# certfhe/CSGN

Hardware: AMD Instinct MI355X
Metric: ciphertext-mults/sec (N=1247, 1024-term operands) (higher is better)
Workload: dtype u64

## Files before the change

csgn_amd/batch.py:

```python
from __future__ import annotations

import ctypes as C
from typing import Optional, Tuple

import numpy as np
import torch

from . import capi
from .capi import check


def _ptr(t: Optional[torch.Tensor]) -> int:
    return 0 if t is None else t.data_ptr()


class HipPath:

    def __init__(self, device: int = 0):
        self.lib = capi.load_library()
        if not torch.cuda.is_available():
            raise capi.CsgnError(capi.CSGN_ERR_NO_DEVICE,
                                 "torch sees no GPU; csgn_amd has no CPU fallback")
        torch.cuda.set_device(device)
        check(self.lib.csgn_init(device))
# ... 775 lines not shown
            out = torch.empty(max(batch, 1), dtype=torch.int64, device=self.device)
        check(self.lib.csgn_uint_decrypt(n_bits, batch, w, h_planes, h_terms, h_off, h_total, h_max, _ptr(mask),
                                         _ptr(out), self.stream))
        return out[:batch]

    def decrypt_combined_uniform(self, n_bits: int, batch: int, t1: int, t2: int, left: torch.Tensor,
                                 right: torch.Tensor, mask: torch.Tensor, product: bool) -> torch.Tensor:
        bits = torch.empty(max(batch, 1), dtype=torch.uint8, device=self.device)
        scratch = torch.empty(int(self.lib.csgn_decrypt_combined_scratch_bytes(batch, t1, t2)),
                              dtype=torch.uint8, device=self.device)
        fn = self.lib.csgn_decrypt_product_uniform if product else self.lib.csgn_decrypt_sum_uniform
        check(fn(n_bits, batch, t1, t2, _ptr(left), _ptr(right), _ptr(mask), _ptr(bits), _ptr(scratch),
                 self.stream))
        return bits[:batch]

    def compact_ragged(self, n_bits: int, words: torch.Tensor, off: torch.Tensor,
                       total_terms: Optional[int] = None, max_terms: int = 0,
                       out: Optional[torch.Tensor] = None, off_out: Optional[torch.Tensor] = None,
                       scratch: Optional[torch.Tensor] = None,
                       sync: bool = True) -> Tuple[torch.Tensor, torch.Tensor]:
        batch = off.numel() - 1
        dl = self.default_len(n_bits)
        if total_terms is None:
            total_terms = int(self.download(off[-1:])[0])
        if out is None:
            out = self.empty_words(max(total_terms * dl, 1))
        if off_out is None:
            off_out = self.empty_words(batch + 1)
        if scratch is None:
            scratch = torch.empty(int(self.lib.csgn_compact_scratch_bytes(n_bits, batch, total_terms)),
# ... 98 lines not shown
```

csgn_amd/capi.py:

```python
from __future__ import annotations

import ctypes as C
import os
from typing import Optional

PKG = os.path.dirname(os.path.abspath(__file__))
_LIB_PATH = os.path.join(PKG, "lib", "libcsgn_hip.so")

CSGN_OK = 0
CSGN_ERR_INVALID = -1
CSGN_ERR_UNSUPPORTED = -2
CSGN_ERR_NO_DEVICE = -3
CSGN_ERR_HIP = -4

CSGN_GATE_NOT, CSGN_GATE_XNOR, CSGN_GATE_NAND, CSGN_GATE_OR, CSGN_GATE_NOR, CSGN_GATE_MUX, \
    CSGN_GATE_ADD_PLAIN, CSGN_GATE_MUL_PLAIN = range(1, 9)

CSGN_UINT_ADD_HALF, CSGN_UINT_ADD_FULL, CSGN_UINT_EQ_STEP, CSGN_UINT_LT_FIRST, CSGN_UINT_LT_STEP = range(1, 6)
CSGN_UINT_PLAIN_EQ, CSGN_UINT_PLAIN_NE, CSGN_UINT_PLAIN_LT, CSGN_UINT_PLAIN_LE, CSGN_UINT_PLAIN_GT, \
    CSGN_UINT_PLAIN_GE = range(1, 7)

u64 = C.c_uint64
vp = C.c_void_p

# ... 35 lines not shown
    "csgn_mul_plan_trust": (C.c_int, [vp, C.c_int]),
    "csgn_mul_ragged_async_plan_words": (u64, [u64]),
    "csgn_mul_ragged_async": (C.c_int, [u64, u64, vp, vp, vp, vp, vp, vp, u64, vp, vp]),
    "csgn_mul_ragged_async_result": (C.c_int, [vp, C.POINTER(u64 * 5), vp]),
    "csgn_add_uniform": (C.c_int, [u64, u64, u64, u64, vp, vp, vp, vp]),
    "csgn_add_ragged": (C.c_int, [u64, u64, vp, vp, vp, vp, vp, vp, u64, vp]),
    "csgn_small_ops": (C.c_int, [u64, u64, vp, vp]),
    "csgn_add_ragged_bounded": (C.c_int, [u64, u64, u64, u64, vp, vp, vp, vp, vp, vp, u64, vp]),
    "csgn_decrypt_scratch_bytes": (C.c_size_t, [u64, u64]),
    "csgn_decrypt_uniform": (C.c_int, [u64, u64, u64, vp, vp, vp, vp, vp]),
    "csgn_decrypt_ragged": (C.c_int, [u64, u64, u64, vp, vp, vp, vp, vp, vp]),
    "csgn_decrypt_ragged_bounded": (C.c_int, [u64, u64, u64, u64, vp, vp, vp, vp, vp, vp]),
    "csgn_decrypt_combined_scratch_bytes": (C.c_size_t, [u64, u64, u64]),
    "csgn_decrypt_product_uniform": (C.c_int, [u64, u64, u64, u64, vp, vp, vp, vp, vp, vp]),
    "csgn_decrypt_sum_uniform": (C.c_int, [u64, u64, u64, u64, vp, vp, vp, vp, vp, vp]),
    "csgn_compact_scratch_bytes": (C.c_size_t, [u64, u64, u64]),
    "csgn_compact_ragged": (C.c_int, [u64, u64, u64, u64, vp, vp, vp, vp, vp, vp]),
    "csgn_encrypt_explicit": (C.c_int, [u64, u64, u64, vp, vp, vp, vp, vp, vp, vp]),
    "csgn_rng_from_os": (C.c_int, [vp, C.c_uint32]),
    "csgn_rng_from_seed": (C.c_int, [vp, u64, C.c_uint32]),
    "csgn_encrypt_keyed_layout": (C.c_int, [u64, C.POINTER(C.c_uint32), C.POINTER(C.c_uint32), C.POINTER(C.c_uint32)]),
    "csgn_encrypt_keyed": (C.c_int, [u64, u64, u64, u64, vp, vp, vp, vp, vp, vp]),
    "csgn_encrypt_mul_keyed": (C.c_int, [u64, u64, u64, u64, vp, vp, vp, vp, vp, vp, vp, vp, vp]),
    "csgn_encrypt_device_rng": (C.c_int, [u64, u64, u64, vp, vp, vp, u64, vp, vp]),
    "csgn_permute_uniform": (C.c_int, [u64, u64, u64, C.c_int, vp, vp, vp, vp]),
    "csgn_bitlen_scratch_bytes": (C.c_size_t, [u64]),
    "csgn_decrypt_bitlen": (C.c_int, [u64, u64, u64, vp, vp, vp, vp, vp, vp]),
    "csgn_permute_bitlen": (C.c_int, [u64, u64, vp, vp, vp, vp, vp, vp]),
    "csgn_synth_fill": (C.c_int, [u64, u64, u64, u64, vp, vp]),
    "csgn_digest": (C.c_int, [vp, u64, u64, vp, vp]),
# ... 2 lines not shown
    "csgn_circuit_input": (C.c_int, [vp, u64, C.POINTER(C.c_uint32)]),
    "csgn_circuit_input_ragged": (C.c_int, [vp, vp, C.POINTER(C.c_uint32)]),
    "csgn_circuit_add": (C.c_int, [vp, C.c_uint32, C.c_uint32, C.POINTER(C.c_uint32)]),
    "csgn_circuit_mul": (C.c_int, [vp, C.c_uint32, C.c_uint32, C.POINTER(C.c_uint32)]),
    "csgn_circuit_decrypt": (C.c_int, [vp, C.c_uint32, vp, C.POINTER(C.c_uint32)]),
    "csgn_circuit_compact": (C.c_int, [vp, C.c_uint32, C.POINTER(C.c_uint32)]),
    "csgn_circuit_permute": (C.c_int, [vp, C.c_uint32, vp, C.POINTER(C.c_uint32)]),
    "csgn_circuit_encrypt": (C.c_int, [vp, u64, vp, vp, vp, vp, u64, C.POINTER(C.c_uint32)]),
    "csgn_circuit_encrypt_mul": (C.c_int, [vp, u64, vp, vp, vp, vp, vp, vp, u64, C.POINTER(C.c_uint32), C.POINTER(C.c_uint32)]),
    "csgn_circuit_epoch": (u64, [vp]),
    "csgn_circuit_node_key": (C.c_int, [vp, vp]),
    "csgn_circuit_optimize": (C.c_int, [vp, C.c_uint32]),
    "csgn_circuit_output": (C.c_int, [vp, C.c_uint32]),
    "csgn_circuit_block_bytes": (u64, [vp]),
    "csgn_circuit_stats": (C.c_int, [vp, vp]),
    "csgn_circuit_plan_json": (C.c_int, [vp, vp, C.c_size_t]),
    "csgn_circuit_build": (C.c_int, [vp]),
    "csgn_circuit_value": (vp, [vp, C.c_uint32]),
    "csgn_circuit_value_terms": (u64, [vp, C.c_uint32]),
    "csgn_circuit_value_total_terms": (u64, [vp, C.c_uint32]),
    "csgn_circuit_value_offsets": (vp, [vp, C.c_uint32]),
    "csgn_circuit_bits": (vp, [vp, C.c_uint32]),
    "csgn_circuit_run": (C.c_int, [vp, vp]),
    "csgn_mul_uniform_kernel": (C.c_char_p, [u64, u64, u64, u64]),
    "csgn_gate_terms": (u64, [C.c_int, u64, u64, u64]),
    "csgn_gate_uniform_kernel": (C.c_char_p, [u64, C.c_int, u64, u64, u64, u64]),
    "csgn_gate_uniform": (C.c_int, [u64, C.c_int, u64, u64, u64, u64, vp, vp, vp, vp, vp, vp]),
    "csgn_const_fill": (C.c_int, [u64, u64, vp, C.c_int, vp, vp]),
    "csgn_uint_step_terms": (u64, [C.c_int, C.c_int, u64, u64, u64]),
    "csgn_uint_step_kernel": (C.c_char_p, [u64, C.c_int, u64, u64, u64, u64]),
# ... 269 lines not shown
```

csgn_amd/csrc/csgn_capi.hip:

```cpp
#include "csgn_capi_util.h"
#include "csgn_device.h"
#include "csgn_tuning.h"

#include <sys/random.h>

#include <cerrno>
#include <cstdarg>
#include <vector>
#include <cstdio>
#include <cstring>

namespace csgn {
namespace capi {

thread_local char g_err[512] = "";

int fail(int code, const char *fmt, ...)
{
    va_list ap;
    va_start(ap, fmt);
    vsnprintf(g_err, sizeof(g_err), fmt, ap);
    va_end(ap);
    return code;
}
// ... 728 lines not shown
    return CSGN_OK;
}

int csgn_decrypt_product_uniform(uint64_t n_bits, uint64_t batch, uint64_t t1, uint64_t t2,
                                 const uint64_t *d_left, const uint64_t *d_right,
                                 const uint64_t *d_mask, uint8_t *d_bits, void *d_scratch, void *stream)
{
    return decrypt_combined_uniform(true, n_bits, batch, t1, t2, d_left, d_right, d_mask, d_bits, d_scratch, stream);
}

int csgn_decrypt_sum_uniform(uint64_t n_bits, uint64_t batch, uint64_t t1, uint64_t t2,
                             const uint64_t *d_left, const uint64_t *d_right,
                             const uint64_t *d_mask, uint8_t *d_bits, void *d_scratch, void *stream)
{
    return decrypt_combined_uniform(false, n_bits, batch, t1, t2, d_left, d_right, d_mask, d_bits, d_scratch, stream);
}

size_t csgn_compact_scratch_bytes(uint64_t n_bits, uint64_t batch, uint64_t total_terms)
{
    if (n_bits == 0 || !csgn::compact_supported(n_bits))
        return 0;
    return csgn::compact_scratch_bytes(n_bits, batch, total_terms);
}

int csgn_compact_ragged(uint64_t n_bits, uint64_t batch, uint64_t total_terms, uint64_t max_terms,
                        const uint64_t *d_terms, const uint64_t *d_off,
                        uint64_t *d_out, uint64_t *d_off_out, void *d_scratch, void *stream)
{
    if (int rc = check_n(n_bits))
        return rc;
// ... 1925 lines not shown
```

csgn_amd/csrc/csgn_circuit.hip:

```cpp
#include "csgn_capi_util.h"

#include <algorithm>
#include <cstring>
#include <map>
#include <string>
#include <vector>

using namespace csgn::capi;

struct csgn_circuit {
    struct Value {
        uint64_t terms = 0;
        std::vector<uint64_t> per;
        uint64_t total = 0;
        uint64_t max_terms = 0;
        bool dynamic = false;
        bool needs_csr = false;
        bool is_input = false;
        bool output = false;
        int producer = -1;
        bool addressable = false;
        bool has_region = false;
        size_t offset = 0;
        uint64_t pitch = 0;
// ... 27 lines not shown
        size_t scratch;
    };
    uint64_t n_bits = 0, batch = 0;
    std::vector<Value> values;
    std::vector<Op> ops;
    std::vector<Expr> exprs;
    std::vector<size_t> bits_offsets;
    uint32_t flags = 0;
    size_t bytes = 0;
    size_t epoch_offset = 0;
    size_t hoist_offset = 0;
    uint32_t n_hoist = 0;
    bool has_encrypt = false;
    uint64_t runs = 0;
    uint64_t stats[8] = {0};
    void *block = nullptr;
    hipGraph_t graph = nullptr;
    hipGraphExec_t exec = nullptr;
};

namespace {

typedef csgn_circuit::Value Value;
typedef csgn_circuit::Op Op;
typedef csgn_circuit::Expr Expr;

uint64_t terms_of(const Value &v, uint64_t i) { return v.per.empty() ? v.terms : v.per[i]; }

Value make_uniform(csgn_circuit *c, uint64_t terms, int producer)
{
// ... 716 lines not shown
                                 (const u64 *)op.mask, base + e.bits, base + e.scratch, s, va.dynamic ? 0 : va.max_terms);
        return csgn::decrypt(c->n_bits, c->batch, va.terms, c->batch * va.terms, A, nullptr, (const u64 *)op.mask,
                             base + e.bits, base + e.scratch, s);
    }
    hipError_t err = emit_expr(c, base, op, e.l, done, alg_bytes, kernels, s);
    if (err == hipSuccess)
        err = emit_expr(c, base, op, e.r, done, alg_bytes, kernels, s);
    if (err != hipSuccess)
        return err;
    *alg_bytes += 3 * c->batch;
    *kernels += 1;
    return csgn::combine_bits(base + c->exprs[(size_t)e.l].bits, base + c->exprs[(size_t)e.r].bits, c->batch, e.kind == 1,
                              base + e.bits, s);
}

}

extern "C" {

int csgn_circuit_build(csgn_circuit *c)
{
    REQUIRE(c && !c->exec, "null circuit, or already built");
    REQUIRE(!c->ops.empty(), "the circuit has no operations");
    if (c->graph) {
        (void)hipGraphDestroy(c->graph);
        c->graph = nullptr;
    }
    if (c->block) {
        (void)hipFree(c->block);
        c->block = nullptr;
// ... 112 lines not shown
        if (op.kind == 6) {
            const Value &vo = c->values[op.out];
            e = va.total ? csgn::compact(c->n_bits, c->batch, va.total, va.max_terms, (const u64 *)A,
                                         reinterpret_cast<const u64 *>(base + va.csr_offset),
                                         reinterpret_cast<u64 *>(base + vo.offset),
                                         reinterpret_cast<u64 *>(base + vo.csr_offset), base + op.scratch, s)
                         : csgn::circuit_zero_words(reinterpret_cast<u64 *>(base + vo.csr_offset), c->batch + 1, s);
            alg += 2 * va.total * dl * 8;
            kernels += 1;
            continue;
        }
        if (op.kind == 2) {
            uint8_t *bits = base + c->bits_offsets[(size_t)op.bits_id];
            if (op.expr >= 0) {
                fused += 1;
                e = emit_expr(c, base, op, op.expr, done, &alg, &kernels, s);
            } else if (!va.per.empty()) {
                e = csgn::decrypt(c->n_bits, c->batch, 0, va.total, (const u64 *)A,
                                  reinterpret_cast<const u64 *>(base + va.csr_offset), (const u64 *)op.mask,
                                  bits, base + op.scratch, s, va.dynamic ? 0 : va.max_terms);
            } else {
                e = csgn::decrypt(c->n_bits, c->batch, va.terms, c->batch * va.terms, (const u64 *)A, nullptr,
                                  (const u64 *)op.mask, bits, base + op.scratch, s);
            }
            if (op.expr < 0) {
                alg += va.total * dl * 8 + c->batch;
                kernels += 1;
            }
            continue;
        }
        const Value &vo = c->values[op.out];
// ... 52 lines not shown
    hipGraph_t g = nullptr;
    const hipError_t e2 = hipStreamEndCapture(s, &g);
    (void)hipStreamDestroy(s);
    if (e != hipSuccess || e2 != hipSuccess) {
        if (g)
            (void)hipGraphDestroy(g);
        return hip_fail(e != hipSuccess ? e : e2, "csgn_circuit_build (stream capture)");
    }
    const hipError_t e3 = hipGraphInstantiate(&c->exec, g, nullptr, nullptr, 0);
    if (e3 != hipSuccess) {
        (void)hipGraphDestroy(g);
        c->exec = nullptr;
        return hip_fail(e3, "hipGraphInstantiate");
    }
    c->graph = g;
    uint64_t regions = 0;
    for (const Value &v : c->values)
        regions += v.has_region ? 1u : 0u;
    c->stats[0] = (uint64_t)c->bytes;
    c->stats[1] = alg;
    c->stats[2] = (uint64_t)c->ops.size();
    c->stats[3] = kernels;
    c->stats[4] = placed;
    c->stats[5] = fused;
    c->stats[6] = dropped;
    (void)regions;
    c->stats[7] = c->n_hoist;
    return CSGN_OK;
}

uint64_t csgn_circuit_block_bytes(const csgn_circuit *c) { return (c && c->block) ? (uint64_t)c->bytes : 0; }

int csgn_circuit_stats(const csgn_circuit *c, uint64_t h_stats[8])
{
    REQUIRE(c && h_stats, "null argument");
    REQUIRE(c->exec, "the circuit is not built");
    for (int i = 0; i < 8; ++i)
        h_stats[i] = c->stats[i];
    return CSGN_OK;
}

int csgn_circuit_plan_json(csgn_circuit *c, char *h_json, size_t cap)
{
    REQUIRE(c && h_json && cap, "null argument");
    REQUIRE(!c->exec, "the circuit is already built");
    REQUIRE(!c->ops.empty(), "the circuit has no operations");
    Compiler comp(c);
    comp.run();
    std::string out = "{\"bytes\": " + std::to_string(c->bytes) + ", \"values\": [";
    for (size_t v = 0; v < c->values.size(); ++v) {
        const Value &val = c->values[v];
        out += std::string(v ? ", " : "") + "{\"region\": " + (val.has_region ? "true" : "false") + ", \"addressable\": " +
               (val.addressable ? "true" : "false") + ", \"offset\": " + std::to_string(val.offset) + ", \"pitch\": " +
               std::to_string(val.pitch) + ", \"parent\": " + std::to_string(val.parent) + ", \"terms\": " +
               std::to_string(val.terms) + ", \"total\": " + std::to_string(val.total) + "}";
    }
// ... 69 lines not shown
```

csgn_amd/csrc/csgn_decrypt.hip:

```cpp
#include "csgn_device.h"

namespace csgn {

namespace {

template <typename Unit>
__global__ void __launch_bounds__(256) k_term_hits(const Unit *__restrict__ terms,
                                                   const Unit *__restrict__ mask, u64 total_terms,
                                                   u32 U, FastDiv dU, u64 *__restrict__ hits,
                                                   u32 *__restrict__ zero4)
{
    extern __shared__ __align__(16) unsigned char smem_raw[];
    if (zero4 && blockIdx.x == 0 && threadIdx.x < 4)
        zero4[threadIdx.x] = 0;
    Unit *lmask = reinterpret_cast<Unit *>(smem_raw);
    u32 *fail = reinterpret_cast<u32 *>(smem_raw + (size_t)U * sizeof(Unit));

    const u32 tid = threadIdx.x;
    const u64 term0 = (u64)blockIdx.x * 256u;
    const u32 nterms = (u32)min((u64)256, total_terms - term0);
    const u32 nunits = nterms * U;
    for (u32 k = tid; k < U; k += 256u)
        lmask[k] = mask[k];
    fail[tid] = 0;
// ... 5 lines not shown
        const Unit x = base[u];
        const u32 t = csgn_fastdiv(u, dU);
        const u32 k = u - t * U;
        if (!unit_covers(x, lmask[k]))
            fail[t] = 1;
    }
    __syncthreads();

    const bool hit = (tid < nterms) && (fail[tid] == 0);
    const u64 b = __ballot(hit);
    if ((tid & (kWave - 1)) == 0)
        hits[(u64)blockIdx.x * 4u + (tid >> 6)] = b;
}

template <typename Unit, int K>
__global__ void __launch_bounds__(256) k_term_hits_seg(const Unit *__restrict__ terms,
                                                       const Unit *__restrict__ mask,
                                                       u64 total_units, u32 U, FastDiv dU, u32 TB,
                                                       unsigned char *__restrict__ hits,
                                                       uint8_t *__restrict__ direct_bits,
                                                       u32 *__restrict__ zero4)
{
    __shared__ u64 ok_bits[K * 4 + 1];
    if (zero4 && blockIdx.x == 0 && threadIdx.x < 4)
        zero4[threadIdx.x] = 0;
    const u32 tid = threadIdx.x, lane = tid & (kWave - 1), wave = tid >> 6;
    const u32 bid = xcd_contiguous_block(blockIdx.x, gridDim.x);
    const u64 g0 = (u64)bid * (256u * K) + tid;

    Unit x[K], mk[K];
    const u64 last = total_units - 1;
#pragma unroll
    for (int j = 0; j < K; ++j) {
        const u64 g = g0 + (u32)j * 256u;
        x[j] = terms[g < last ? g : last];
    }
#pragma unroll
    for (int j = 0; j < K; ++j) {
        const u32 local = (u32)j * 256u + tid;
        mk[j] = mask[local - csgn_fastdiv(local, dU) * U];
    }
#pragma unroll
// ... 25 lines not shown
            const u32 first = t;
            const u32 nbits = min(64u, TB - first);
            unsigned char *dst = hits + (u64)bid * (TB >> 3) + (first >> 3);
            if (nbits == 64u)
                *reinterpret_cast<u64 *>(dst) = hb;
            else if (nbits == 32u)
                *reinterpret_cast<u32 *>(dst) = (u32)hb;
            else if (nbits == 16u)
                *reinterpret_cast<unsigned short *>(dst) = (unsigned short)hb;
            else
                *dst = (unsigned char)hb;
        }
    }
}

constexpr u64 kChunkTerms = 65536;

struct LongWork {
    u32 *counters;
    u32 *slot_ct;
    u32 *slot_par;
    u32 *slot_left;
    u64 *entries;
};

template <int G, int MODE>
__global__ void __launch_bounds__(256) k_hits_parity(const u64 *__restrict__ hits,
                                                     const u64 *__restrict__ off, u64 T, u64 batch,
                                                     uint8_t *__restrict__ bits, LongWork work)
{
    const u64 gid = (u64)blockIdx.x * 256u + threadIdx.x;
// ... 17 lines not shown
    u32 par = 0;
    if (e > s) {
        const u64 w0 = s >> 6, w1 = (e - 1) >> 6;
        for (u64 w = w0 + lane; w <= w1; w += G) {
            u64 x = hits[w];
            if (w == w0)
                x &= ~0ull << (s & 63);
            if (w == w1 && (e & 63))
                x &= (1ull << (e & 63)) - 1;
            par ^= (u32)__popcll(x);
        }
    }
    if (G == 1) {
        bits[b] = (uint8_t)(par & 1u);
    } else {
        const u64 odd = __ballot(par & 1u);
        if (lane == 0)
            bits[b] = (uint8_t)(__popcll(odd) & 1);
    }
}

__global__ void __launch_bounds__(256) k_hits_parity_chunks(const u64 *__restrict__ hits,
                                                            const u64 *__restrict__ off, LongWork work,
                                                            uint8_t *__restrict__ bits)
{
    __shared__ u32 wave_par[4];
    const u32 n = work.counters[1];
    for (u32 i = blockIdx.x; i < n; i += gridDim.x) {
        const u64 ent = work.entries[i];
        const u32 slot = (u32)(ent >> 32), c = (u32)ent;
        const u32 b = work.slot_ct[slot];
        const u64 s = off[b], e = off[b + 1];
        const u64 cs = s + (u64)c * kChunkTerms, ce = min(e, cs + kChunkTerms);
        const u64 w0 = cs >> 6, w1 = (ce - 1) >> 6;
// ... 70 lines not shown
static size_t decrypt_bitmap_bytes(u64 total_terms)
{
    return (size_t)((total_terms + 255) / 256) * 32u + 64u;
}

static u64 decrypt_max_long(u64 batch, u64 total_terms)
{
    const u64 by_terms = total_terms / (kLongTerms + 1) + 1;
    return batch < by_terms ? batch : by_terms;
}
static u64 decrypt_max_entries(u64 batch, u64 total_terms)
{
    return decrypt_max_long(batch, total_terms) + total_terms / kChunkTerms + 1;
}

size_t decrypt_scratch_bytes(u64 batch, u64 total_terms)
{
    const size_t uniform = (size_t)batch * 4u + 16u;
    const size_t ragged = 16u + (size_t)decrypt_max_long(batch, total_terms) * 12u + 8u +
                          (size_t)decrypt_max_entries(batch, total_terms) * 8u;
    return decrypt_bitmap_bytes(total_terms) + (uniform > ragged ? uniform : ragged);
}

hipError_t decrypt(u64 n_bits, u64 batch, u64 terms_uniform, u64 total_terms, const u64 *terms,
                   const u64 *off, const u64 *mask, uint8_t *bits, void *scratch, hipStream_t s, u64 max_terms)
{
    const u64 dL = (n_bits + 63) / 64;
    if (batch == 0)
        return hipSuccess;
    if (off && max_terms != 0 && batch * max_terms == total_terms) {
// ... 8 lines not shown
        work.counters = reinterpret_cast<u32 *>(wbase);
        work.slot_ct = work.counters + 4;
        work.slot_par = work.slot_ct + max_long;
        work.slot_left = work.slot_par + max_long;
        work.entries = reinterpret_cast<u64 *>(wbase + ((16u + max_long * 12u + 7u) & ~(size_t)7u));
    }
    u32 *zero4 = work.counters;
    if (total_terms) {
        const bool wide = (dL % 2 == 0) && aligned16(terms) && aligned16(mask);
        const u32 U = (u32)(wide ? dL / 2 : dL);
        const u64 blocks64 = (total_terms + 255) / 256;
        if (blocks64 > kMaxBlocks256)
            return hipErrorInvalidValue;
        const u32 blocks = (u32)blocks64;
        const FastDiv dU = csgn_fastdiv_make(U);
        int k_seg = 0;
        if (U <= 64u)
            for (int k = 1; k <= 8; ++k)
                if ((256u * k) % U == 0 && ((256u * k) / U) % 8u == 0) {
                    k_seg = k;
                    break;
                }
        if (k_seg && tune(TUNE_DEC_LOOP) == 0) {
            const u32 tb = 256u * k_seg / U;
            const u64 nblk = (total_terms + tb - 1) / tb;
            if (nblk > kMaxBlocks256)
                return hipErrorInvalidValue;
            unsigned char *hb = reinterpret_cast<unsigned char *>(scratch);
            const u64 tu = total_terms * U;
            uint8_t *direct = (!off && terms_uniform == 1) ? bits : nullptr;
#define CSGN_HITS_SEG(K)                                                                              \
    do {                                                                                              \
        if (wide)                                                                                     \
            k_term_hits_seg<unit16, K><<<(u32)nblk, 256, 0, s>>>(                                     \
                reinterpret_cast<const unit16 *>(terms), reinterpret_cast<const unit16 *>(mask), tu, U, \
                dU, tb, hb, direct, zero4);                                                           \
        else                                                                                          \
// ... 20 lines not shown
            k_term_hits<unit8><<<blocks, 256, (size_t)U * 8 + 1024, s>>>(terms, mask, total_terms, U,
                                                                        dU, hits, zero4);
        hipError_t e = hipGetLastError();
        if (e != hipSuccess)
            return e;
    }
    if (off) {
        if (batch >= (1ull << 32))
            return hipErrorInvalidValue;
        k_hits_parity<1, 1><<<ceil_div_u64(batch, 256), 256, 0, s>>>(hits, off, 0, batch, bits, work);
        if (total_terms > kLongTerms && (max_terms == 0 || max_terms > kLongTerms)) {
            const u64 max_entries = decrypt_max_entries(batch, total_terms);
            k_hits_parity_chunks<<<(u32)std::min<u64>(8192, max_entries), 256, 0, s>>>(hits, off, work, bits);
        }
    } else if (terms_uniform <= kLongTerms) {
        k_hits_parity<1, 0><<<ceil_div_u64(batch, 256), 256, 0, s>>>(hits, nullptr, terms_uniform, batch, bits, LongWork{});
    } else if (batch * ((terms_uniform + 65535) / 65536) <= kMaxBlocks256) {
        u32 *partial = reinterpret_cast<u32 *>(reinterpret_cast<unsigned char *>(scratch) +
                                               decrypt_bitmap_bytes(total_terms));
        hipError_t e = zero_words(reinterpret_cast<u64 *>(partial), (batch + 1) / 2, s);
        if (e != hipSuccess)
            return e;
        const u32 chunks = (u32)((terms_uniform + 65535) / 65536);
        k_hits_parity_chunked<<<(u32)(batch * chunks), 256, 0, s>>>(hits, terms_uniform, chunks, partial);
        k_partial_to_bits<<<ceil_div_u64(batch, 256), 256, 0, s>>>(partial, batch, bits);
    } else {
        if (batch * 64 > kMaxBlocks256 * 256u)
            return hipErrorInvalidValue;
        k_hits_parity<64, 0><<<ceil_div_u64(batch * 64, 256), 256, 0, s>>>(hits, nullptr, terms_uniform, batch, bits, LongWork{});
    }
    return hipGetLastError();
// ... 26 lines not shown
}

hipError_t decrypt_combined(u64 n_bits, u64 batch, u64 t1, u64 t2, const u64 *L, const u64 *R,
                            const u64 *mask, bool is_product, uint8_t *bits, void *scratch, hipStream_t s)
{
    if (batch == 0)
        return hipSuccess;
    const size_t pad = 256;
    auto up = [&](size_t x) { return (x + pad - 1) / pad * pad; };
    unsigned char *base = reinterpret_cast<unsigned char *>(scratch);
    base = reinterpret_cast<unsigned char *>(up(reinterpret_cast<uintptr_t>(base)));
    unsigned char *s1 = base;
    unsigned char *s2 = s1 + up(decrypt_scratch_bytes(batch, batch * t1));
    uint8_t *b1 = s2 + up(decrypt_scratch_bytes(batch, batch * t2));
    uint8_t *b2 = b1 + up(batch);
    hipError_t e = decrypt(n_bits, batch, t1, batch * t1, L, nullptr, mask, b1, s1, s);
    if (e != hipSuccess)
        return e;
    e = decrypt(n_bits, batch, t2, batch * t2, R, nullptr, mask, b2, s2, s);
    if (e != hipSuccess)
        return e;
    k_combine_bits<<<ceil_div_u64(batch, 256), 256, 0, s>>>(b1, b2, batch, is_product ? 1 : 0, bits);
    return hipGetLastError();
}

}
```

csgn_amd/csrc/csgn_kernels.h:

```cpp
#pragma once

#include "csgn_common.h"

#include <vector>

struct csgn_small_op;

namespace csgn {

struct MulTuning {
    int m;
    int ti;
    int nt;
    int flat;
    int bs;
    int xcd;
};
MulTuning mul_tuning();
const char *mul_uniform_kernel_name(u64 n_bits, u64 pairs, u64 t1, u64 t2);

hipError_t mul_uniform(u64 n_bits, u64 batch, u64 t1, u64 t2, const u64 *L, const u64 *R, u64 *out,
                       u64 out_slots, hipStream_t s, u64 out_pitch_words = 0);
u64 mul_ragged_plan_scratch_words(u64 batch);
u64 mul_ragged_plan_head_words();
// ... 277 lines not shown
hipError_t uint_write(u64 n_bits, u64 batch, u64 v, const u64 *const *index, const u64 *s, u64 rows, u64 w,
                      const u64 *const *value, const u64 *tv, const u64 *const *arrays, const u64 *td, u64 *const *out,
                      hipStream_t stream);

enum ScratchSlot { SCRATCH_UINT_PLAIN, SCRATCH_UINT_LUT, SCRATCH_UINT_READ, SCRATCH_UINT_ADDK, SCRATCH_UINT_FIND, SCRATCH_GATHER, SCRATCH_MATMUL, SCRATCH_COUNT, SCRATCH_UINT_LT_SELECT, SCRATCH_UINT_PICK, SCRATCH_UINT_WRITE, SCRATCH_UINT_ARITH, SCRATCH_UINT_PICK_ROWS, SCRATCH_SLOTS };
u64 *scratch_take(ScratchSlot slot, size_t bytes, hipStream_t s, bool &owned, hipError_t &e);
hipError_t scratch_done(u64 *block, bool owned, hipError_t e);
void scratch_stats(u64 out[5]);

hipError_t small_ops(u64 n_bits, u64 count, const ::csgn_small_op *ops, hipStream_t s);
size_t decrypt_scratch_bytes(u64 batch, u64 total_terms);
hipError_t combine_bits(const uint8_t *a, const uint8_t *b, u64 n, bool is_product, uint8_t *out, hipStream_t s);
size_t decrypt_combined_scratch_bytes(u64 batch, u64 t1, u64 t2);
hipError_t decrypt_combined(u64 n_bits, u64 batch, u64 t1, u64 t2, const u64 *L, const u64 *R,
                            const u64 *mask, bool is_product, uint8_t *bits, void *scratch, hipStream_t s);

constexpr u32 kUintDecryptMaxPlanes = 64;
const char *uint_decrypt_kernel_name(u64 n_bits, u64 batch, u64 n_planes, const u64 *terms);
hipError_t uint_decrypt(u64 n_bits, u64 batch, u64 n_planes, const u64 *const *planes, const u64 *terms,
                        const u64 *const *off, const u64 *max_terms, const u64 *mask, u64 *values, hipStream_t stream);

}
```

include/csgn_hip.h:

```cpp
#ifndef CSGN_HIP_H
#define CSGN_HIP_H

#include <stddef.h>
#include <stdint.h>

#ifdef __cplusplus
extern "C" {
#endif

typedef enum csgn_status {
    CSGN_OK = 0,
    CSGN_ERR_INVALID = -1,
    CSGN_ERR_UNSUPPORTED = -2,
    CSGN_ERR_NO_DEVICE = -3,
    CSGN_ERR_HIP = -4
} csgn_status;

#define CSGN_ABI_VERSION 1


int csgn_abi_version(void);
const char *csgn_last_error(void);

int csgn_init(int device);
// ... 87 lines not shown
                         uint8_t *d_bits, void *d_scratch, void *stream);
int csgn_decrypt_ragged(uint64_t n_bits, uint64_t batch, uint64_t total_terms,
                        const uint64_t *d_terms, const uint64_t *d_off, const uint64_t *d_mask,
                        uint8_t *d_bits, void *d_scratch, void *stream);
int csgn_decrypt_ragged_bounded(uint64_t n_bits, uint64_t batch, uint64_t total_terms, uint64_t max_terms,
                                const uint64_t *d_terms, const uint64_t *d_off, const uint64_t *d_mask,
                                uint8_t *d_bits, void *d_scratch, void *stream);

size_t csgn_decrypt_combined_scratch_bytes(uint64_t batch, uint64_t t1, uint64_t t2);
int csgn_decrypt_product_uniform(uint64_t n_bits, uint64_t batch, uint64_t t1, uint64_t t2,
                                 const uint64_t *d_left, const uint64_t *d_right,
                                 const uint64_t *d_mask, uint8_t *d_bits, void *d_scratch, void *stream);
int csgn_decrypt_sum_uniform(uint64_t n_bits, uint64_t batch, uint64_t t1, uint64_t t2,
                             const uint64_t *d_left, const uint64_t *d_right,
                             const uint64_t *d_mask, uint8_t *d_bits, void *d_scratch, void *stream);

size_t csgn_compact_scratch_bytes(uint64_t n_bits, uint64_t batch, uint64_t total_terms);
int csgn_compact_ragged(uint64_t n_bits, uint64_t batch, uint64_t total_terms, uint64_t max_terms,
                        const uint64_t *d_terms, const uint64_t *d_off,
                        uint64_t *d_out, uint64_t *d_off_out, void *d_scratch, void *stream);


int csgn_encrypt_explicit(uint64_t n_bits, uint64_t d, uint64_t batch,
                          const uint8_t *d_plain, const uint64_t *d_rnd,
                          const uint32_t *d_chosen, const uint8_t *d_last,
                          const uint64_t *d_mask, uint64_t *d_out, void *stream);
typedef struct csgn_rng {
    uint32_t key[8];
    uint64_t nonce;
    uint32_t rounds;
// ... 50 lines not shown
                             const uint64_t *d_key, const uint64_t *d_mask, const csgn_rng *h_rng_a,
                             const csgn_rng *h_rng_b, uint64_t first_ciphertext, uint32_t *value, uint32_t *bits_id);
uint64_t csgn_circuit_epoch(const csgn_circuit *circuit);
int csgn_circuit_node_key(const csgn_rng *h_rng, uint32_t h_node_key[8]);
#define CSGN_CIRCUIT_REUSE 1u
#define CSGN_CIRCUIT_PLACE 2u
#define CSGN_CIRCUIT_FUSE_DECRYPT 4u
#define CSGN_CIRCUIT_PUSHDOWN 8u
#define CSGN_CIRCUIT_HOIST 16u
#define CSGN_CIRCUIT_ALL 23u
int csgn_circuit_optimize(csgn_circuit *circuit, uint32_t flags);
int csgn_circuit_output(csgn_circuit *circuit, uint32_t value);
int csgn_circuit_build(csgn_circuit *circuit);
uint64_t csgn_circuit_block_bytes(const csgn_circuit *circuit);
int csgn_circuit_stats(const csgn_circuit *circuit, uint64_t h_stats[8]);
int csgn_circuit_plan_json(csgn_circuit *circuit, char *h_json, size_t cap);
uint64_t *csgn_circuit_value(csgn_circuit *circuit, uint32_t value);
uint64_t csgn_circuit_value_terms(csgn_circuit *circuit, uint32_t value);
uint64_t csgn_circuit_value_total_terms(csgn_circuit *circuit, uint32_t value);
const uint64_t *csgn_circuit_value_offsets(csgn_circuit *circuit, uint32_t value);
uint8_t *csgn_circuit_bits(csgn_circuit *circuit, uint32_t bits_id);
int csgn_circuit_run(csgn_circuit *circuit, void *stream);

const char *csgn_mul_uniform_kernel(uint64_t n_bits, uint64_t pairs, uint64_t t1, uint64_t t2);


enum {
    CSGN_GATE_NOT = 1,
    CSGN_GATE_XNOR,
    CSGN_GATE_NAND,
// ... 275 lines not shown
```

Measured before the change: 45680.

## Fuse decrypt expression trees into two kernel launches

Adds a generic expression-decrypt path. It computes term hits for all leaves in one multi-leaf kernel, then evaluates per-batch parity and the xor/and program in a single kernel, replacing per-leaf decrypts plus combine launches. The circuit builder and the combined product/sum decrypt now route through this path, and a launch-count query API is added. The metric is ciphertext multiplication throughput, so this decrypt-side change likely does not touch the measured path.

```diff
diff --git a/csgn_amd/batch.py b/csgn_amd/batch.py
--- a/csgn_amd/batch.py
+++ b/csgn_amd/batch.py
@@ -813,6 +813,19 @@
                  self.stream))
         return bits[:batch]
 
+    def decrypt_expr_uniform(self, n_bits: int, batch: int, leaves, terms, mask: torch.Tensor, program) -> torch.Tensor:
+        nl, nn = len(leaves), len(program)
+        assert nl == len(terms)
+        h_leaves = (C.c_void_p * max(nl, 1))(*[None if p is None else _ptr(p) for p in leaves])
+        h_terms = (C.c_uint64 * max(nl, 1))(*[int(t) for t in terms])
+        h_prog = (C.c_uint32 * max(3 * nn, 1))(*[int(x) for node in program for x in node])
+        bits = torch.empty(max(batch, 1), dtype=torch.uint8, device=self.device)
+        scratch = torch.empty(max(int(self.lib.csgn_decrypt_expr_scratch_bytes(batch, nl, h_terms, nn)), 1),
+                              dtype=torch.uint8, device=self.device)
+        check(self.lib.csgn_decrypt_expr_uniform(n_bits, batch, nl, h_leaves, h_terms, _ptr(mask), nn, h_prog,
+                                                 _ptr(bits), _ptr(scratch), self.stream))
+        return bits[:batch]
+
     def compact_ragged(self, n_bits: int, words: torch.Tensor, off: torch.Tensor,
                        total_terms: Optional[int] = None, max_terms: int = 0,
                        out: Optional[torch.Tensor] = None, off_out: Optional[torch.Tensor] = None,
diff --git a/csgn_amd/capi.py b/csgn_amd/capi.py
--- a/csgn_amd/capi.py
+++ b/csgn_amd/capi.py
@@ -73,6 +73,8 @@
     "csgn_decrypt_combined_scratch_bytes": (C.c_size_t, [u64, u64, u64]),
     "csgn_decrypt_product_uniform": (C.c_int, [u64, u64, u64, u64, vp, vp, vp, vp, vp, vp]),
     "csgn_decrypt_sum_uniform": (C.c_int, [u64, u64, u64, u64, vp, vp, vp, vp, vp, vp]),
+    "csgn_decrypt_expr_scratch_bytes": (C.c_size_t, [u64, u64, vp, u64]),
+    "csgn_decrypt_expr_uniform": (C.c_int, [u64, u64, u64, vp, vp, vp, u64, vp, vp, vp, vp]),
     "csgn_compact_scratch_bytes": (C.c_size_t, [u64, u64, u64]),
     "csgn_compact_ragged": (C.c_int, [u64, u64, u64, u64, vp, vp, vp, vp, vp, vp]),
     "csgn_encrypt_explicit": (C.c_int, [u64, u64, u64, vp, vp, vp, vp, vp, vp, vp]),
@@ -105,6 +107,7 @@
     "csgn_circuit_output": (C.c_int, [vp, C.c_uint32]),
     "csgn_circuit_block_bytes": (u64, [vp]),
     "csgn_circuit_stats": (C.c_int, [vp, vp]),
+    "csgn_circuit_launches": (u64, [vp]),
     "csgn_circuit_plan_json": (C.c_int, [vp, vp, C.c_size_t]),
     "csgn_circuit_build": (C.c_int, [vp]),
     "csgn_circuit_value": (vp, [vp, C.c_uint32]),
diff --git a/csgn_amd/csrc/csgn_capi.hip b/csgn_amd/csrc/csgn_capi.hip
--- a/csgn_amd/csrc/csgn_capi.hip
+++ b/csgn_amd/csrc/csgn_capi.hip
@@ -766,6 +766,61 @@
                              const uint64_t *d_mask, uint8_t *d_bits, void *d_scratch, void *stream)
 {
     return decrypt_combined_uniform(false, n_bits, batch, t1, t2, d_left, d_right, d_mask, d_bits, d_scratch, stream);
+}
+
+constexpr uint64_t kExprMaxLeaves = 32, kExprMaxNodes = 32;
+
+size_t csgn_decrypt_expr_scratch_bytes(uint64_t batch, uint64_t n_leaves, const uint64_t *h_terms, uint64_t n_nodes)
+{
+    if (n_leaves == 0 || n_leaves > kExprMaxLeaves || n_nodes > kExprMaxNodes || !h_terms)
+        return 0;
+    return csgn::decrypt_expr_scratch_bytes(batch, (u32)n_leaves, (const u64 *)h_terms, (u32)n_nodes);
+}
+
+int csgn_decrypt_expr_uniform(uint64_t n_bits, uint64_t batch, uint64_t n_leaves, const uint64_t *const *h_leaves,
+                              const uint64_t *h_terms, const uint64_t *d_mask, uint64_t n_nodes,
+                              const uint32_t *h_program, uint8_t *d_bits, void *d_scratch, void *stream)
+{
+    if (int rc = check_n(n_bits))
+        return rc;
+    REQUIRE(n_leaves >= 1 && n_leaves <= kExprMaxLeaves, "decrypt_expr: %llu leaves (1 .. %llu)",
+            (unsigned long long)n_leaves, (unsigned long long)kExprMaxLeaves);
+    REQUIRE(n_nodes <= kExprMaxNodes, "decrypt_expr: %llu nodes (at most %llu)", (unsigned long long)n_nodes,
+            (unsigned long long)kExprMaxNodes);
+    REQUIRE(h_leaves && h_terms && (h_program || n_nodes == 0), "null host pointer");
+    for (uint64_t i = 0; i < n_nodes; ++i) {
+        const uint32_t *p = h_program + 3 * i;
+        REQUIRE(p[0] <= 1u, "decrypt_expr: node %llu: operation %u (0 = xor, 1 = and)", (unsigned long long)i, p[0]);
+        REQUIRE(p[1] < n_leaves + i && p[2] < n_leaves + i,
+                "decrypt_expr: node %llu reads values %u and %u: children precede parents (below %llu)",
+                (unsigned long long)i, p[1], p[2], (unsigned long long)(n_leaves + i));
+    }
+    const uint64_t dl = csgn_default_len(n_bits);
+    for (uint64_t i = 0; i < n_leaves; ++i)
+        if (!product_below(batch, h_terms[i], dl, 1ull << 60))
+            return fail(CSGN_ERR_UNSUPPORTED, "decrypt_expr: leaf %llu: batch of %llu x %llu terms: size overflows",
+                        (unsigned long long)i, (unsigned long long)batch, (unsigned long long)h_terms[i]);
+    REQUIRE(d_mask && d_bits && d_scratch, "null device pointer");
+    for (uint64_t i = 0; i < n_leaves; ++i)
+        REQUIRE(h_leaves[i] || h_terms[i] == 0, "null device pointer (leaf %llu)", (unsigned long long)i);
+    if (batch == 0)
+        return CSGN_OK;
+    const size_t pad = 256;
+    auto up = [&](size_t x) { return (x + pad - 1) / pad * pad; };
+    unsigned char *at = reinterpret_cast<unsigned char *>(up(reinterpret_cast<uintptr_t>(d_scratch)));
+    csgn::ExprLeaf leaves[kExprMaxLeaves];
+    csgn::ExprNode nodes[kExprMaxNodes];
+    for (uint64_t i = 0; i < n_leaves; ++i) {
+        leaves[i] = csgn::ExprLeaf{(const u64 *)h_leaves[i], h_terms[i], at, nullptr};
+        at += up(csgn::decrypt_scratch_bytes(batch, batch * h_terms[i]));
+    }
+    for (uint64_t i = 0; i < n_leaves; ++i, at += up((size_t)batch))
+        leaves[i].bits = at;
+    for (uint64_t i = 0; i < n_nodes; ++i, at += up((size_t)batch))
+        nodes[i] = csgn::ExprNode{h_program[3 * i] == 1u, h_program[3 * i + 1], h_program[3 * i + 2], at};
+    HIP_TRY(csgn::decrypt_expr(n_bits, batch, (u32)n_leaves, leaves, (const u64 *)d_mask, (u32)n_nodes, nodes, d_bits,
+                               S(stream)));
+    return CSGN_OK;
 }
 
 size_t csgn_compact_scratch_bytes(uint64_t n_bits, uint64_t batch, uint64_t total_terms)
diff --git a/csgn_amd/csrc/csgn_circuit.hip b/csgn_amd/csrc/csgn_circuit.hip
--- a/csgn_amd/csrc/csgn_circuit.hip
+++ b/csgn_amd/csrc/csgn_circuit.hip
@@ -65,6 +65,7 @@
     bool has_encrypt = false;
     uint64_t runs = 0;
     uint64_t stats[8] = {0};
+    uint64_t launches = 0;
     void *block = nullptr;
     hipGraph_t graph = nullptr;
     hipGraphExec_t exec = nullptr;
@@ -811,6 +812,62 @@
                               base + e.bits, s);
 }
 
+hipError_t emit_expr_fused(csgn_circuit *c, unsigned char *base, const Op &op, std::vector<char> &done, uint64_t *alg_bytes,
+                           uint64_t *kernels, hipStream_t s, bool *fused)
+{
+    *fused = false;
+    std::vector<int> order, index(c->exprs.size(), -1);
+    std::vector<std::pair<int, int>> stack(1, std::make_pair(op.expr, 0));
+    std::vector<char> seen(c->exprs.size(), 0);
+    while (!stack.empty()) {
+        const int ei = stack.back().first, phase = stack.back().second;
+        const Expr &e = c->exprs[(size_t)ei];
+        if (phase == 0 && seen[(size_t)ei]) {
+            stack.pop_back();
+            continue;
+        }
+        seen[(size_t)ei] = 1;
+        if (e.kind < 0 || phase == 2) {
+            order.push_back(ei);
+            stack.pop_back();
+            continue;
+        }
+        stack.back().second = phase + 1;
+        stack.push_back(std::make_pair(phase == 0 ? e.l : e.r, 0));
+    }
+    std::vector<csgn::ExprLeaf> leaves;
+    std::vector<csgn::ExprNode> nodes;
+    for (int ei : order) {
+        const Expr &e = c->exprs[(size_t)ei];
+        if (e.kind >= 0)
+            continue;
+        const Value &va = c->values[e.value];
+        if (!va.per.empty())
+            return hipSuccess;
+        index[(size_t)ei] = (int)leaves.size();
+        leaves.push_back(csgn::ExprLeaf{reinterpret_cast<const u64 *>(base + va.offset), va.terms, base + e.scratch, base + e.bits});
+    }
+    for (int ei : order) {
+        const Expr &e = c->exprs[(size_t)ei];
+        if (e.kind < 0)
+            continue;
+        index[(size_t)ei] = (int)(leaves.size() + nodes.size());
+        nodes.push_back(csgn::ExprNode{e.kind == 1, (u32)index[(size_t)e.l], (u32)index[(size_t)e.r], base + e.bits});
+    }
+    if (!csgn::decrypt_expr_fused(c->n_bits, c->batch, (u32)leaves.size(), leaves.data(), (const u64 *)op.mask, (u32)nodes.size()))
+        return hipSuccess;
+    const uint64_t dl = csgn_default_len(c->n_bits);
+    for (int ei : order) {
+        const Expr &e = c->exprs[(size_t)ei];
+        done[(size_t)ei] = 1;
+        *alg_bytes += e.kind < 0 ? c->values[e.value].total * dl * 8 + c->batch : 3 * c->batch;
+        *kernels += 1;
+    }
+    *fused = true;
+    return csgn::decrypt_expr(c->n_bits, c->batch, (u32)leaves.size(), leaves.data(), (const u64 *)op.mask, (u32)nodes.size(),
+                              nodes.data(), base + c->exprs[(size_t)op.expr].bits, s);
+}
+
 }
 
 extern "C" {
@@ -953,7 +1010,10 @@
             uint8_t *bits = base + c->bits_offsets[(size_t)op.bits_id];
             if (op.expr >= 0) {
                 fused += 1;
-                e = emit_expr(c, base, op, op.expr, done, &alg, &kernels, s);
+                bool two_launches = false;
+                e = emit_expr_fused(c, base, op, done, &alg, &kernels, s, &two_launches);
+                if (e == hipSuccess && !two_launches)
+                    e = emit_expr(c, base, op, op.expr, done, &alg, &kernels, s);
             } else if (!va.per.empty()) {
                 e = csgn::decrypt(c->n_bits, c->batch, 0, va.total, (const u64 *)A,
                                   reinterpret_cast<const u64 *>(base + va.csr_offset), (const u64 *)op.mask,
@@ -1036,6 +1096,8 @@
         return hip_fail(e3, "hipGraphInstantiate");
     }
     c->graph = g;
+    size_t graph_nodes = 0;
+    c->launches = hipGraphGetNodes(g, nullptr, &graph_nodes) == hipSuccess ? (uint64_t)graph_nodes : 0;
     uint64_t regions = 0;
     for (const Value &v : c->values)
         regions += v.has_region ? 1u : 0u;
@@ -1062,6 +1124,8 @@
     return CSGN_OK;
 }
 
+uint64_t csgn_circuit_launches(const csgn_circuit *c) { return (c && c->exec) ? c->launches : 0; }
+
 int csgn_circuit_plan_json(csgn_circuit *c, char *h_json, size_t cap)
 {
     REQUIRE(c && h_json && cap, "null argument");
diff --git a/csgn_amd/csrc/csgn_decrypt.hip b/csgn_amd/csrc/csgn_decrypt.hip
--- a/csgn_amd/csrc/csgn_decrypt.hip
+++ b/csgn_amd/csrc/csgn_decrypt.hip
@@ -43,18 +43,12 @@
 }
 
 template <typename Unit, int K>
-__global__ void __launch_bounds__(256) k_term_hits_seg(const Unit *__restrict__ terms,
-                                                       const Unit *__restrict__ mask,
-                                                       u64 total_units, u32 U, FastDiv dU, u32 TB,
-                                                       unsigned char *__restrict__ hits,
-                                                       uint8_t *__restrict__ direct_bits,
-                                                       u32 *__restrict__ zero4)
-{
-    __shared__ u64 ok_bits[K * 4 + 1];
-    if (zero4 && blockIdx.x == 0 && threadIdx.x < 4)
-        zero4[threadIdx.x] = 0;
+__device__ __forceinline__ void term_hits_seg_block(const Unit *__restrict__ terms, const Unit *__restrict__ mask,
+                                                    u64 total_units, u32 U, FastDiv dU, u32 TB,
+                                                    unsigned char *__restrict__ hits,
+                                                    uint8_t *__restrict__ direct_bits, u32 bid, u64 *ok_bits)
+{
     const u32 tid = threadIdx.x, lane = tid & (kWave - 1), wave = tid >> 6;
-    const u32 bid = xcd_contiguous_block(blockIdx.x, gridDim.x);
     const u64 g0 = (u64)bid * (256u * K) + tid;
 
     Unit x[K], mk[K];
@@ -110,7 +104,80 @@
     }
 }
 
+template <typename Unit, int K>
+__global__ void __launch_bounds__(256) k_term_hits_seg(const Unit *__restrict__ terms,
+                                                       const Unit *__restrict__ mask,
+                                                       u64 total_units, u32 U, FastDiv dU, u32 TB,
+                                                       unsigned char *__restrict__ hits,
+                                                       uint8_t *__restrict__ direct_bits,
+                                                       u32 *__restrict__ zero4)
+{
+    __shared__ u64 ok_bits[K * 4 + 1];
+    if (zero4 && blockIdx.x == 0 && threadIdx.x < 4)
+        zero4[threadIdx.x] = 0;
+    const u32 bid = xcd_contiguous_block(blockIdx.x, gridDim.x);
+    term_hits_seg_block<Unit, K>(terms, mask, total_units, U, dU, TB, hits, direct_bits, bid, ok_bits);
+}
+
+constexpr u32 kExprLeaves = 32;
+constexpr u32 kExprValues = 64;
+constexpr u32 kExprGroup = 16;
+constexpr u64 kGroupTerms = 320;
+
+struct ExprLeafTable {
+    const void *terms[kExprLeaves];
+    unsigned char *hits[kExprLeaves];
+    u64 units[kExprLeaves];
+    u64 T[kExprLeaves];
+    u32 first[kExprLeaves];
+    u32 n;
+};
+
+struct ExprProgram {
+    unsigned char kind[kExprValues], l[kExprValues], r[kExprValues];
+    u32 n;
+};
+
+template <typename Unit, int K, int NL>
+__global__ void __launch_bounds__(256) k_term_hits_leaves(ExprLeafTable t, const Unit *__restrict__ mask, u32 U,
+                                                          FastDiv dU, u32 TB)
+{
+    __shared__ u64 ok_bits[K * 4 + 1];
+    const u32 g = xcd_contiguous_block(blockIdx.x, gridDim.x);
+    if (NL <= 4) {
+        const void *terms = t.terms[0];
+        unsigned char *hits = t.hits[0];
+        u64 units = t.units[0];
+        u32 first = 0;
+#pragma unroll
+        for (int i = 1; i < NL; ++i) {
+            const bool in = t.first[i] <= g;
+            terms = in ? t.terms[i] : terms;
+            hits = in ? t.hits[i] : hits;
+            units = in ? t.units[i] : units;
+            first = in ? t.first[i] : first;
+        }
+        term_hits_seg_block<Unit, K>(reinterpret_cast<const Unit *>(terms), mask, units, U, dU, TB, hits, nullptr,
+                                     g - first, ok_bits);
+        return;
+    }
+    u32 leaf = 0;
+    for (u32 i = 1; i < t.n; ++i)
+        leaf += (t.first[i] <= g) ? 1u : 0u;
+    term_hits_seg_block<Unit, K>(reinterpret_cast<const Unit *>(t.terms[leaf]), mask, t.units[leaf], U, dU, TB,
+                                 t.hits[leaf], nullptr, g - t.first[leaf], ok_bits);
+}
+
 constexpr u64 kChunkTerms = 65536;
+
+template <int G>
+__device__ __forceinline__ u64 group_bits(u64 ballot)
+{
+    if (G >= 64)
+        return ballot;
+    const u32 first = (threadIdx.x & (kWave - 1)) & ~(u32)(G - 1);
+    return (ballot >> first) & ((1ull << (G & 63)) - 1ull);
+}
 
 struct LongWork {
     u32 *counters;
@@ -158,10 +225,48 @@
     if (G == 1) {
         bits[b] = (uint8_t)(par & 1u);
     } else {
-        const u64 odd = __ballot(par & 1u);
+        const u64 odd = group_bits<G>(__ballot(par & 1u));
         if (lane == 0)
             bits[b] = (uint8_t)(__popcll(odd) & 1);
     }
+}
+
+__global__ void __launch_bounds__(256) k_expr_parity(ExprLeafTable t, ExprProgram prog, u64 batch,
+                                                     uint8_t *__restrict__ bits)
+{
+    const u64 gid = (u64)blockIdx.x * 256u + threadIdx.x;
+    const u64 b = gid / kExprGroup;
+    const u32 lane = (u32)(gid % kExprGroup);
+    if (b >= batch)
+        return;
+    u64 val = 0;
+    for (u32 i = 0; i < t.n; ++i) {
+        const u64 T = t.T[i];
+        const u64 *__restrict__ hits = reinterpret_cast<const u64 *>(t.hits[i]);
+        const u64 s = b * T, e = s + T;
+        u32 par = 0;
+        if (e > s) {
+            const u64 w0 = s >> 6, w1 = (e - 1) >> 6;
+            for (u64 w = w0 + lane; w <= w1; w += kExprGroup) {
+                u64 x = hits[w];
+                if (w == w0)
+                    x &= ~0ull << (s & 63);
+                if (w == w1 && (e & 63))
+                    x &= (1ull << (e & 63)) - 1;
+                par ^= (u32)__popcll(x);
+            }
+        }
+        const u64 odd = group_bits<kExprGroup>(__ballot(par & 1u));
+        val |= (u64)(__popcll(odd) & 1) << i;
+    }
+    u32 last = t.n - 1;
+    for (u32 i = 0; i < prog.n; ++i) {
+        const u64 l = (val >> prog.l[i]) & 1u, r = (val >> prog.r[i]) & 1u;
+        last = t.n + i;
+        val |= (prog.kind[i] ? (l & r) : (l ^ r)) << last;
+    }
+    if (lane == 0)
+        bits[b] = (uint8_t)((val >> last) & 1u);
 }
 
 __global__ void __launch_bounds__(256) k_hits_parity_chunks(const u64 *__restrict__ hits,
@@ -262,6 +367,15 @@
     return decrypt_max_long(batch, total_terms) + total_terms / kChunkTerms + 1;
 }
 
+static int decrypt_seg_k(u32 U)
+{
+    if (U <= 64u)
+        for (int k = 1; k <= 8; ++k)
+            if ((256u * k) % U == 0 && ((256u * k) / U) % 8u == 0)
+                return k;
+    return 0;
+}
+
 size_t decrypt_scratch_bytes(u64 batch, u64 total_terms)
 {
     const size_t uniform = (size_t)batch * 4u + 16u;
@@ -300,13 +414,7 @@
             return hipErrorInvalidValue;
         const u32 blocks = (u32)blocks64;
         const FastDiv dU = csgn_fastdiv_make(U);
-        int k_seg = 0;
-        if (U <= 64u)
-            for (int k = 1; k <= 8; ++k)
-                if ((256u * k) % U == 0 && ((256u * k) / U) % 8u == 0) {
-                    k_seg = k;
-                    break;
-                }
+        const int k_seg = decrypt_seg_k(U);
         if (k_seg && tune(TUNE_DEC_LOOP) == 0) {
             const u32 tb = 256u * k_seg / U;
             const u64 nblk = (total_terms + tb - 1) / tb;
@@ -357,7 +465,10 @@
             k_hits_parity_chunks<<<(u32)std::min<u64>(8192, max_entries), 256, 0, s>>>(hits, off, work, bits);
         }
     } else if (terms_uniform <= kLongTerms) {
-        k_hits_parity<1, 0><<<ceil_div_u64(batch, 256), 256, 0, s>>>(hits, nullptr, terms_uniform, batch, bits, LongWork{});
+        if (terms_uniform > kGroupTerms && batch * kExprGroup <= kMaxBlocks256 * 256u)
+            k_hits_parity<(int)kExprGroup, 0><<<ceil_div_u64(batch * kExprGroup, 256), 256, 0, s>>>(hits, nullptr, terms_uniform, batch, bits, LongWork{});
+        else
+            k_hits_parity<1, 0><<<ceil_div_u64(batch, 256), 256, 0, s>>>(hits, nullptr, terms_uniform, batch, bits, LongWork{});
     } else if (batch * ((terms_uniform + 65535) / 65536) <= kMaxBlocks256) {
         u32 *partial = reinterpret_cast<u32 *>(reinterpret_cast<unsigned char *>(scratch) +
                                                decrypt_bitmap_bytes(total_terms));
@@ -414,14 +525,127 @@
     unsigned char *s2 = s1 + up(decrypt_scratch_bytes(batch, batch * t1));
     uint8_t *b1 = s2 + up(decrypt_scratch_bytes(batch, batch * t2));
     uint8_t *b2 = b1 + up(batch);
-    hipError_t e = decrypt(n_bits, batch, t1, batch * t1, L, nullptr, mask, b1, s1, s);
-    if (e != hipSuccess)
-        return e;
-    e = decrypt(n_bits, batch, t2, batch * t2, R, nullptr, mask, b2, s2, s);
-    if (e != hipSuccess)
-        return e;
-    k_combine_bits<<<ceil_div_u64(batch, 256), 256, 0, s>>>(b1, b2, batch, is_product ? 1 : 0, bits);
+    const ExprLeaf leaves[2] = {{L, t1, s1, b1}, {R, t2, s2, b2}};
+    const ExprNode node = {is_product, 0, 1, nullptr};
+    return decrypt_expr(n_bits, batch, 2, leaves, mask, 1, &node, bits, s);
+}
+
+bool decrypt_expr_fused(u64 n_bits, u64 batch, u32 n_leaves, const ExprLeaf *leaves, const u64 *mask, u32 n_nodes)
+{
+    const u64 dL = (n_bits + 63) / 64;
+    if (n_leaves == 0 || n_leaves > kExprLeaves || (u64)n_leaves + n_nodes > kExprValues)
+        return false;
+    if (batch * kExprGroup > kMaxBlocks256 * 256u)
+        return false;
+    const bool even = dL % 2 == 0;
+    if (even && !aligned16(mask))
+        return false;
+    const u32 U = (u32)(even ? dL / 2 : dL);
+    const int k = decrypt_seg_k(U);
+    if (!k || tune(TUNE_DEC_LOOP) != 0)
+        return false;
+    const u32 tb = 256u * (u32)k / U;
+    u64 blocks = 0;
+    for (u32 i = 0; i < n_leaves; ++i) {
+        if (leaves[i].t > kLongTerms)
+            return false;
+        if (even && !aligned16(leaves[i].terms))
+            return false;
+        blocks += (batch * leaves[i].t + tb - 1) / tb;
+        if (blocks > kMaxBlocks256)
+            return false;
+    }
+    return true;
+}
+
+hipError_t decrypt_expr(u64 n_bits, u64 batch, u32 n_leaves, const ExprLeaf *leaves, const u64 *mask, u32 n_nodes,
+                        const ExprNode *nodes, uint8_t *bits, hipStream_t s)
+{
+    if (batch == 0 || n_leaves == 0)
+        return hipSuccess;
+    if (!decrypt_expr_fused(n_bits, batch, n_leaves, leaves, mask, n_nodes)) {
+        for (u32 i = 0; i < n_leaves; ++i) {
+            uint8_t *out = (n_nodes == 0 && i == n_leaves - 1) ? bits : leaves[i].bits;
+            const hipError_t e = decrypt(n_bits, batch, leaves[i].t, batch * leaves[i].t, leaves[i].terms, nullptr, mask,
+                                         out, leaves[i].scratch, s);
+            if (e != hipSuccess)
+                return e;
+        }
+        auto value = [&](u32 v) { return v < n_leaves ? leaves[v].bits : nodes[v - n_leaves].bits; };
+        for (u32 i = 0; i < n_nodes; ++i) {
+            const hipError_t e = combine_bits(value(nodes[i].l), value(nodes[i].r), batch, nodes[i].is_and,
+                                              i == n_nodes - 1 ? bits : nodes[i].bits, s);
+            if (e != hipSuccess)
+                return e;
+        }
+        return hipSuccess;
+    }
+    const u64 dL = (n_bits + 63) / 64;
+    const bool wide = dL % 2 == 0;
+    const u32 U = (u32)(wide ? dL / 2 : dL);
+    const int k_seg = decrypt_seg_k(U);
+    const u32 tb = 256u * (u32)k_seg / U;
+    const FastDiv dU = csgn_fastdiv_make(U);
+    ExprLeafTable t = {};
+    ExprProgram prog = {};
+    u64 blocks = 0;
+    for (u32 i = 0; i < n_leaves; ++i) {
+        t.terms[i] = leaves[i].terms;
+        t.hits[i] = reinterpret_cast<unsigned char *>(leaves[i].scratch);
+        t.units[i] = batch * leaves[i].t * U;
+        t.T[i] = leaves[i].t;
+        t.first[i] = (u32)blocks;
+        blocks += (batch * leaves[i].t + tb - 1) / tb;
+    }
+    t.n = n_leaves;
+    for (u32 i = n_leaves; i < kExprLeaves; ++i)
+        t.first[i] = ~0u;
+    const bool few = n_leaves <= 4;
+    for (u32 i = 0; i < n_nodes; ++i) {
+        prog.kind[i] = nodes[i].is_and ? 1 : 0;
+        prog.l[i] = (unsigned char)nodes[i].l;
+        prog.r[i] = (unsigned char)nodes[i].r;
+    }
+    prog.n = n_nodes;
+    if (blocks) {
+#define CSGN_HITS_LEAVES(K)                                                                                        \
+    do {                                                                                                           \
+        if (wide && few)                                                                                           \
+            k_term_hits_leaves<unit16, K, 4><<<(u32)blocks, 256, 0, s>>>(t, reinterpret_cast<const unit16 *>(mask), U, dU, tb); \
+        else if (wide)                                                                                             \
+            k_term_hits_leaves<unit16, K, 32><<<(u32)blocks, 256, 0, s>>>(t, reinterpret_cast<const unit16 *>(mask), U, dU, tb); \
+        else if (few)                                                                                              \
+            k_term_hits_leaves<unit8, K, 4><<<(u32)blocks, 256, 0, s>>>(t, mask, U, dU, tb);                       \
+        else                                                                                                       \
+            k_term_hits_leaves<unit8, K, 32><<<(u32)blocks, 256, 0, s>>>(t, mask, U, dU, tb);                      \
+    } while (0)
+        switch (k_seg) {
+        case 1: CSGN_HITS_LEAVES(1); break;
+        case 2: CSGN_HITS_LEAVES(2); break;
+        case 3: CSGN_HITS_LEAVES(3); break;
+        case 4: CSGN_HITS_LEAVES(4); break;
+        case 5: CSGN_HITS_LEAVES(5); break;
+        case 6: CSGN_HITS_LEAVES(6); break;
+        case 7: CSGN_HITS_LEAVES(7); break;
+        default: CSGN_HITS_LEAVES(8); break;
+        }
+#undef CSGN_HITS_LEAVES
+        const hipError_t e = hipGetLastError();
+        if (e != hipSuccess)
+            return e;
+    }
+    k_expr_parity<<<ceil_div_u64(batch * kExprGroup, 256), 256, 0, s>>>(t, prog, batch, bits);
     return hipGetLastError();
 }
 
-}
+size_t decrypt_expr_scratch_bytes(u64 batch, u32 n_leaves, const u64 *terms, u32 n_nodes)
+{
+    const size_t pad = 256;
+    auto up = [&](size_t x) { return (x + pad - 1) / pad * pad; };
+    size_t n = pad;
+    for (u32 i = 0; i < n_leaves; ++i)
+        n += up(decrypt_scratch_bytes(batch, batch * terms[i]));
+    return n + ((size_t)n_leaves + n_nodes) * up((size_t)batch);
+}
+
+}
diff --git a/csgn_amd/csrc/csgn_kernels.h b/csgn_amd/csrc/csgn_kernels.h
--- a/csgn_amd/csrc/csgn_kernels.h
+++ b/csgn_amd/csrc/csgn_kernels.h
@@ -315,6 +315,21 @@
 size_t decrypt_combined_scratch_bytes(u64 batch, u64 t1, u64 t2);
 hipError_t decrypt_combined(u64 n_bits, u64 batch, u64 t1, u64 t2, const u64 *L, const u64 *R,
                             const u64 *mask, bool is_product, uint8_t *bits, void *scratch, hipStream_t s);
+struct ExprLeaf {
+    const u64 *terms;
+    u64 t;
+    void *scratch;
+    uint8_t *bits;
+};
+struct ExprNode {
+    bool is_and;
+    u32 l, r;
+    uint8_t *bits;
+};
+bool decrypt_expr_fused(u64 n_bits, u64 batch, u32 n_leaves, const ExprLeaf *leaves, const u64 *mask, u32 n_nodes);
+hipError_t decrypt_expr(u64 n_bits, u64 batch, u32 n_leaves, const ExprLeaf *leaves, const u64 *mask, u32 n_nodes,
+                        const ExprNode *nodes, uint8_t *bits, hipStream_t s);
+size_t decrypt_expr_scratch_bytes(u64 batch, u32 n_leaves, const u64 *terms, u32 n_nodes);
 
 constexpr u32 kUintDecryptMaxPlanes = 64;
 const char *uint_decrypt_kernel_name(u64 n_bits, u64 batch, u64 n_planes, const u64 *terms);
diff --git a/include/csgn_hip.h b/include/csgn_hip.h
--- a/include/csgn_hip.h
+++ b/include/csgn_hip.h
@@ -125,6 +125,11 @@
 int csgn_decrypt_sum_uniform(uint64_t n_bits, uint64_t batch, uint64_t t1, uint64_t t2,
                              const uint64_t *d_left, const uint64_t *d_right,
                              const uint64_t *d_mask, uint8_t *d_bits, void *d_scratch, void *stream);
+
+size_t csgn_decrypt_expr_scratch_bytes(uint64_t batch, uint64_t n_leaves, const uint64_t *h_terms, uint64_t n_nodes);
+int csgn_decrypt_expr_uniform(uint64_t n_bits, uint64_t batch, uint64_t n_leaves, const uint64_t *const *h_leaves,
+                              const uint64_t *h_terms, const uint64_t *d_mask, uint64_t n_nodes,
+                              const uint32_t *h_program, uint8_t *d_bits, void *d_scratch, void *stream);
 
 size_t csgn_compact_scratch_bytes(uint64_t n_bits, uint64_t batch, uint64_t total_terms);
 int csgn_compact_ragged(uint64_t n_bits, uint64_t batch, uint64_t total_terms, uint64_t max_terms,
@@ -205,6 +210,7 @@
 int csgn_circuit_build(csgn_circuit *circuit);
 uint64_t csgn_circuit_block_bytes(const csgn_circuit *circuit);
 int csgn_circuit_stats(const csgn_circuit *circuit, uint64_t h_stats[8]);
+uint64_t csgn_circuit_launches(const csgn_circuit *circuit);
 int csgn_circuit_plan_json(csgn_circuit *circuit, char *h_json, size_t cap);
 uint64_t *csgn_circuit_value(csgn_circuit *circuit, uint32_t value);
 uint64_t csgn_circuit_value_terms(csgn_circuit *circuit, uint32_t value);
```

Result: slower. 45060 (-1.4%).
